# smu-ivpl/FastInterCU-VVC

Hardware: AMD Instinct MI355X
Metric: CU-inferences/sec (batch 4096, 128x128) (higher is better)
Workload: dtype f16 (fp32 accumulate)

## Files before the change

fastintercu-vvc_amd/csrc/mlt_chain_kernel.inc:

```
template <class T> __device__ __forceinline__ T karg_reload(size_t off) {
  const __attribute__((address_space(4))) char *ka = (const __attribute__((address_space(4))) char *)__builtin_amdgcn_kernarg_segment_ptr();
  asm volatile("" : "+s"(ka));
  return *(const __attribute__((address_space(4))) T *)(ka + off);
}
#define KARG(type, member) karg_reload<type>(offsetof(ChainArgs, member))

template <int C, int HL, int SPW_L, int WCB, int WPB, int WAVES_C, int WAVES_P, int GT, int RB, int FD, int MINW, int NCONV, bool SPLIT_ROLES, bool S2 = false, bool KEEP = true, bool OOBZ = false, bool W2 = false, bool LO8 = false>
__global__ __launch_bounds__(64 * WAVES_C * WAVES_P, MINW) void chain_kernel(const ChainArgs a) {
  constexpr int KC = 64, NCHUNK = C / KC, KS = KC / 16, SLOTS = KC / 8, TAPS = 9, NG = (TAPS + GT - 1) / GT, GT_LAST = TAPS - (NG - 1) * GT;
  constexpr int CBT = WCB * WAVES_C, CT = 32 * CBT, NPASS = C / CT, NW = WAVES_C * WAVES_P;
  constexpr int H = 1 << HL, HW = H * H, M = HW << SPW_L;
  static_assert(C % CT == 0 && NPASS <= 2 && M == 32 * WAVES_P * WPB && HW >= 32 && C % KC == 0, "tiling");
  static_assert(GT_LAST == GT || RB == 2, "a shorter last tap group issues fewer ring pieces: only with the uncounted vmcnt(0) wait of a 2-deep ring");
  constexpr int WP = (W2 && !LO8) ? 2 : 1, WPLANE = GT * KS * CBT * 1024;
  constexpr int WLO8 = LO8 ? GT * CBT * 2048 : 0;
  constexpr int WCHUNK = WP * WPLANE + WLO8, NPIECE = WCHUNK / 1024, NBUF = RB, PFD = RB - 1;
  static_assert(!W2 || (!S2 && GT_LAST == GT), "hi+lo weights: no stride-2 front conv, whole tap groups");
  static_assert(!LO8 || (W2 && KS == 4 && FD == 1 && KEEP && NCHUNK > 1), "FP8 lo plane: 64-channel chunks, fragment reads one item ahead, stage forms");
  constexpr int REGION8 = LO8 ? M * KC : 0, ACT8 = NCHUNK * REGION8;
  constexpr int NWR = SPLIT_ROLES ? NW / 2 : NW, NWP = SPLIT_ROLES ? NW - NWR : NW, WP0 = SPLIT_ROLES ? NWR : 0;
  constexpr int PPWR = (NPIECE + NWR - 1) / NWR;
  constexpr int REGION = M * KC * 2, ACT = NCHUNK * REGION, RPIECE = REGION / 1024, PPR = (RPIECE + NWP - 1) / NWP;
  constexpr int A8BASE = ACT + NBUF * WCHUNK;
  static_assert(A8BASE + ACT8 <= 160 * 1024, "LDS");
  static_assert(RB >= 2 && RB <= 4, "ring depth");
  static_assert(SPLIT_ROLES || RB == 2, "unified issue waits with vmcnt(0)");
  static_assert(!S2 || KEEP, "the whole-stage variant keeps sc / b0 in registers");
  static_assert(FD >= 1 && FD <= 3 && FD * (WP * WCB + WPB) + (LO8 ? 2 * (WCB > WPB ? WCB : WPB) : 0) <= 15, "fragment prefetch distance");
  static_assert((WP - 1) * WPLANE + ((GT * KS - 1) * CBT + WCB - 1) * 1024 < 65536 && WPLANE + WLO8 < 65536, "fragment offsets are ds_read immediates");
  constexpr int CIN = C / 2, HIN = 2 * H, KCS = 16, NCS = CIN / KCS, TAPS_S = 10, NS = S2 ? NPASS * NCS : 0;
  constexpr int NCH = NCONV * NPASS * NCHUNK * NG;
  constexpr int WSTEP_S = TAPS_S * CBT * 1024, NPIECE_S = WSTEP_S / 1024;
  constexpr int PRS = 2 * H + 1, PCW = 2 * H + 1, PPS = PRS * PCW, PPIX = PPS << SPW_L;
  constexpr int PBYTES = (PPIX * KCS * 2 + 1023) / 1024 * 1024, PPIECE = PBYTES / 1024;
  constexpr int SOFF0 = ACT + 8 * 1024, SOFF1 = ACT + WCHUNK + 8 * 1024;
  constexpr int NPB = 3 * PBYTES <= SOFF0 ? 3 : 2, PLA = NPB - 1;
  auto pbuf = [](int i) { return NPB == 3 ? i % 3 : (i + 1) & 1; };
  static_assert(!S2 || (NPB == 3 ? (NS - 1) % 3 == 0 : (NS - 1) % 2 == 1), "S2: the last stride-2 step must read patch buffer 0");
  static_assert(!S2 || (SPLIT_ROLES && RB == 2 && NS % 2 == 0 && NCH % 2 == 0 && (NCS - 1) % 2 == 1), "S2: step parities");
  static_assert(!S2 || (2 * PBYTES <= SOFF0 && SOFF0 + WSTEP_S <= ACT + WCHUNK && SOFF1 + WSTEP_S <= 160 * 1024), "S2: LDS layout");

  extern __shared__ __attribute__((aligned(16))) char smem[];
  char *ring = smem + ACT;
  const uint32_t lds0 = (uint32_t)(uintptr_t)LDS_PTR(smem);
  const int tid = threadIdx.x, lane = tid & 63;
  const int wave = __builtin_amdgcn_readfirstlane(tid >> 6);
  const int wc = wave % WAVES_C, wp = wave / WAVES_C;
  const int p = lane & 31, h = lane >> 5;
  const bool ring_wave = wave < NWR, patch_wave = wave >= WP0;
  const int lane16 = lane * 16;

  const int pr = p < 4 ? p : p < 12 ? p + 12 : p < 16 ? p - 8 : p < 20 ? p + 8 : p < 28 ? p - 12 : p;
  int mj[WPB], pj[WPB];
// ... 23 lines not shown
  };

  const int ntiles = (a.n + (1 << SPW_L) - 1) >> SPW_L;
  int t = blockIdx.x;
  const int tstep = gridDim.x;
  if (t >= ntiles) return;

  int steps_to_issue = ((ntiles - 1 - t) / tstep + 1) * (NS + NCH);
  int r_pos = 0, r_cv = 0, r_ps = 0, r_ci = 0, r_gi = 0, ahead = 0;
  int slot_wr = 0;
  auto issue_ring = [&]() {
    if (steps_to_issue <= 0) return;
    const bool s_step = S2 && r_pos < NS;
    if (ring_wave) {
      if (s_step) {
      } else {
        const char *wsrc = (const char *)(r_cv == 0 ? a.cv[0].w : r_cv == 1 ? a.cv[1].w : a.cv[NCONV > 2 ? 2 : 1].w);
        const char *src = wsrc + (size_t)((r_ps * NCHUNK + r_ci) * TAPS + r_gi * GT) * (KS * CBT * 1024);
        char *dst = ring + slot_wr * WCHUNK;
        const int npiece = (GT_LAST != GT && r_gi == NG - 1) ? GT_LAST * KS * CBT : NPIECE;
        const size_t wlo = W2 ? (r_cv == 0 ? a.cv[0].w_lo_off : r_cv == 1 ? a.cv[1].w_lo_off : a.cv[NCONV > 2 ? 2 : 1].w_lo_off) : 0;
#pragma unroll
        for (int k = 0; k < PPWR; ++k) {
          int pi = wave + k * NWR;
          pi = pi < npiece ? pi : npiece - 1;
          const int pl = W2 ? pi / (WPLANE / 1024) : 0, pw = W2 ? pi - pl * (WPLANE / 1024) : pi;
          if (LO8 && pl) glds16(wsrc + wlo + (size_t)((r_ps * NCHUNK + r_ci) * TAPS + r_gi * GT) * (CBT * 2048) + pw * 1024 + lane16, dst + pi * 1024);
          else glds16(src + (pl ? wlo : 0) + pw * 1024 + lane16, dst + pi * 1024);
        }
      }
    }
    if (s_step) {
      const char *src = (const char *)a.s2_w + (size_t)r_pos * WSTEP_S;
      char *dst = smem + ((r_pos & 1) ? SOFF1 : SOFF0);
#pragma unroll
      for (int k = 0; k < (NPIECE_S + NW - 1) / NW; ++k) {
        const int pi = wave + k * NW;
        if (pi < NPIECE_S) glds16(src + pi * 1024 + lane16, dst + pi * 1024);
      }
    }
    --steps_to_issue;
    ++ahead;
    if (!s_step) {
      if (++slot_wr == NBUF) slot_wr = 0;
      if (++r_gi == NG) { r_gi = 0; if (++r_ci == NCHUNK) { r_ci = 0; if (++r_ps == NPASS) { r_ps = 0; if (++r_cv == NCONV) r_cv = 0; } } }
    }
    if (++r_pos == NS + NCH) r_pos = 0;
  };
  constexpr int PPW = (PPIECE + NW - 1) / NW;
  uint32_t pvo[S2 ? PPW : 1];
  if constexpr (S2) {
#pragma unroll
    for (int k = 0; k < PPW; ++k) {
      const int piece = wave + k * NW;
      const int it = piece * 64 + lane, qS = it >> 1, pos = it & 1;
      const int sl = pos ^ ((qS >> 3) & 1);
      const int sm = qS / PPS, rem = qS - sm * PPS, r = rem / PCW, kk = rem - r * PCW;
      const int ri = r - 1, ci = kk <= H ? 2 * kk - 1 : 2 * (kk - H - 1);
      const bool live = qS < PPIX && ri >= 0 && ri < HIN && ci >= 0 && ci < HIN;
      const uint32_t off = a.x_c16 ? ((ri * HIN + ci) * KCS + sl * 8) * 2
// ... 126 lines not shown
      if (patch_wave) asm volatile("s_waitcnt vmcnt(0)" ::: "memory");
      PHC_MARK(1);
      asm volatile("s_barrier" ::: "memory");
      PHC_MARK(0);
    }
    if constexpr (S2) {
      asm volatile("s_waitcnt vmcnt(0)\n\ts_barrier" ::: "memory");
      PHC_MARK(0);
      int bS[WPB];
#pragma unroll
      for (int j = 0; j < WPB; ++j) bS[j] = ((pj[j] >> (2 * HL)) * PRS + 2 * ((pj[j] >> HL) & (H - 1))) * PCW + (pj[j] & (H - 1));
      auto put_t = [&](int pass, int i, int j, int qq, uint4v w) {
        const int cb = pass * CT + (wc * WCB + i) * 32 + 16 * qq + 8 * h;
        *(uint4v *)(smem + (cb / KC) * REGION + pj[j] * (KC * 2) + ((((cb % KC) / 8) ^ swz(pj[j])) << 4)) = w;
      };
      static_for<NPASS>([&](auto kp) {
        constexpr int ps = decltype(kp)::value;
        float16v acc[WCB][WPB], accs[WCB][WPB];
#pragma unroll
        for (int i = 0; i < WCB; ++i)
#pragma unroll
          for (int j = 0; j < WPB; ++j)
#pragma unroll
            for (int r = 0; r < 16; ++r) { acc[i][j][r] = 0.f; accs[i][j][r] = 0.f; }
#pragma unroll 1
        for (int chunk = 0; chunk < NCS; ++chunk) {
          const int si = ps * NCS + chunk;
          if (si >= 1 && si + PLA < NS) patch_dma(t, si + PLA);
          issue_ring();
          {
// ... 75 lines not shown
              for (int qq = 0; qq < 2; ++qq) put_t(0, i, j, qq, hold0[i][j][qq]);
        }
      });
      asm volatile("s_waitcnt lgkmcnt(0)\n\ts_barrier" ::: "memory");
      PHC_MARK(3);
    }

    static_for<NCONV>([&](auto kc) {
      constexpr int cvi = decltype(kc)::value;
      constexpr bool lastc = cvi == NCONV - 1;
      const ChainConv &cv = a.cv[cvi];
      constexpr int RES = NCONV == 3 ? (cvi == 0 ? (S2 ? 2 : 1) : cvi == 2 ? (KEEP ? 2 : 1) : 0) : (cvi == 1 ? 1 : 0);
      constexpr bool SAVE = KEEP && NCONV == 3 && cvi == 0;
      constexpr bool RES_LATE = !KEEP;
      uint4v hold[WCB][WPB][2];
      static_for<NPASS>([&](auto kp) {
        constexpr int ps = decltype(kp)::value;
        constexpr bool last = lastc && ps == NPASS - 1;
        float16v acc[WCB][WPB];
#pragma unroll
        for (int i = 0; i < WCB; ++i)
#pragma unroll
          for (int j = 0; j < WPB; ++j)
#pragma unroll
            for (int r = 0; r < 16; ++r) acc[i][j][r] = 0.f;
        uint4v resv[WCB][WPB][2];

#pragma unroll 1
        for (int chunk = 0; chunk < NCHUNK; ++chunk) {
          const uint32_t pl = lds0 + chunk * REGION;
// ... 157 lines not shown
          };
#pragma unroll 1
          for (int g = 0; g < (GT_LAST != GT ? NG - 1 : NG); ++g) do_step(g, std::integral_constant<int, GT * KS>{});
          if constexpr (GT_LAST != GT) do_step(NG - 1, std::integral_constant<int, GT_LAST * KS>{});
        }
        if constexpr (lastc) {
          if constexpr (last) {
            if constexpr (S2) {
              if (has_next) {
#pragma unroll
                for (int i = 0; i < NPB; ++i) patch_dma(t + tstep, i);
              }
            } else if (has_next) dma_region(t + tstep, NCHUNK - 1);
          }
          if constexpr (S2 || !KEEP) out_index_late();
          auto std_epi = [&]() {
          float4v bq[WCB][4], bsq[1][4];
#pragma unroll
          for (int i = 0; i < WCB; ++i) {
            if constexpr (PBIAS) bias_rows(pb_cv[cvi][ps], i, bq[i]);
            else {
#pragma unroll
              for (int q = 0; q < 4; ++q) bq[i][q] = *(const float4v *)(cv.bias + ps * CT + (wc * WCB + i) * 32 + 4 * h + 8 * q);
            }
          }
          ConvArgs ea{};
          ea.y = a.y; ea.gap = a.gap; ea.gap_slots = a.gap_slots; ea.gap_l = a.gap_l; ea.acc_scale = cv.acc_scale; ea.relu = 1;
          ea.y_c16 = a.y_c16; ea.hout_l = HL;
          ea.res = RES ? (const void *)a.x : nullptr;
          float16v acc_sc[1][1];
          uint4v resl[1][1][2];
          if constexpr (RES == 2) {
#pragma unroll
            for (int i = 0; i < WCB; ++i)
#pragma unroll
              for (int j = 0; j < WPB; ++j)
#pragma unroll
                for (int qq = 0; qq < 2; ++qq) resv[i][j][qq] = keep[ps][i][j][qq];
          }
          int he = h, pe = p;
          asm volatile("" : "+v"(he), "+v"(pe));
          conv_epilogue<C, CT, WCB, WPB, false, 1>(ea, ps, wc, he, pe, opix, gidx, acc, acc_sc, bq, bsq, resv, resl);
          };
          auto blk_epi = [&]() {
            ConvArgs ea{};
            ea.y = KARG(void *, y); ea.gap = KARG(float *, gap); ea.gap_slots = KARG(int, gap_slots); ea.gap_l = KARG(int, gap_l);
            ea.acc_scale = KARG(float, cv[cvi].acc_scale); ea.relu = 1;
            ea.y_c16 = KARG(int, y_c16); ea.hout_l = HL;
            ea.res = RES ? (const void *)ea.y : nullptr;
            float16v acc_sc[1][1];
            uint4v resl[1][1][2];
            float4v bsq[1][4];
#pragma unroll
            for (int i = 0; i < WCB; ++i) {
              float4v bq1[1][4];
              bias_rows(pb_cv[cvi][ps], i, bq1[0]);
              if (i) out_index_late();
              int he = h, pe = p;
              asm volatile("" : "+v"(he), "+v"(pe));
              conv_epilogue<C, CT, 1, WPB, false, 1>(ea, ps, wc * WCB + i, he, pe, opix, gidx, reinterpret_cast<float16v(&)[1][WPB]>(acc[i]), acc_sc, bq1, bsq,
                                                     reinterpret_cast<const uint4v(&)[1][WPB][2]>(resv[i]), resl);
            }
          };
          if constexpr (!KEEP && PBIAS) blk_epi();
          else std_epi();
          PHC_MARK(6 + 3 * cvi);
        } else {
          _Float16 *yb0 = nullptr;
          if constexpr (!KEEP) yb0 = (_Float16 *)KARG(void *, cv[cvi].y);
          const int hm = KEEP ? h : (int)__builtin_amdgcn_mbcnt_hi(~0u, __builtin_amdgcn_mbcnt_lo(~0u, 0u)) >> 5;
          auto put = [&](int pass, int i, int j, int qq, uint4v w) {
            const int cb = pass * CT + (wc * WCB + i) * 32 + 16 * qq + 8 * hm;
            *(uint4v *)(smem + (cb / KC) * REGION + pj[j] * (KC * 2) + ((((cb % KC) / 8) ^ swz(pj[j])) << 4)) = w;
            if constexpr (LO8) {
              uint32_t d0, d1;
              cvt_frag_fp8(*(const half8 *)&w, d0, d1);
              typedef uint32_t uint2v __attribute__((ext_vector_type(2)));
              *(uint2v *)(smem + A8BASE + (cb / KC) * REGION8 + pj[j] * KC + (((((cb % KC) >> 4) ^ ((pj[j] >> 2) & 3)) << 4) | (cb & 8))) = uint2v{d0, d1};
            }
          };
// ... 28 lines not shown
              for (int i = 0; i < WCB; ++i)
#pragma unroll
                for (int j = 0; j < WPB; ++j)
#pragma unroll
                  for (int qq = 0; qq < 2; ++qq) put(0, i, j, qq, hold[i][j][qq]);
            }
            asm volatile("s_waitcnt lgkmcnt(0)\n\ts_barrier" ::: "memory");
          }
          PHC_MARK(6 + 3 * cvi);
        }
      });
    });
  }
  PHC_FLUSH((C == 256 ? 2 : 0) + (S2 ? 1 : 0));
}
```

fastintercu-vvc_amd/csrc/mlt_dispatch.cpp:

```cpp
#include "mlt_runtime.h"

const char *tuning_env(const char *name) {
  const char *e = std::getenv("MLT_TUNING");
  return (e && e[0] == '1') ? std::getenv(name) : nullptr;
}

const Tuning &tuning() {
  static const Tuning t = [] {
    auto num = [](const char *name, long dflt) { const char *e = tuning_env(name); return e ? std::atol(e) : dflt; };
    auto on = [](const char *name) { return tuning_env(name) != nullptr; };
    auto cap = [&](const char *name) { const long v = num(name, 0); return (int)(v > 0 ? v : 256); };
    Tuning u{};
    u.debug_dump_dir = tuning_env("MLT_DEBUG_DUMP_DIR");
    u.xl_kill = (int)num("MLT_XL_KILL", 0); u.xl_kill_layer = (int)num("MLT_XL_KILL_LAYER", -1);
    u.lat_pixels = num("MLT_LAT_PIXELS", 16384L);
    u.no_exact_lat = on("MLT_NO_EXACT_LAT"); u.exact_patch_big = !on("MLT_EXACT_PATCH_64K");
    u.wg_cap = cap("MLT_WG_CAP"); u.wg_cap0 = cap("MLT_WG_CAP0"); u.wg_cap1 = cap("MLT_WG_CAP1"); u.wg_cap2 = cap("MLT_WG_CAP2");
    u.l0_mfma32 = on("MLT_L0_MFMA32"); u.l1_mfma32 = !on("MLT_L1_MFMA16");
    u.no_block_fusion = on("MLT_NO_BLOCK_FUSION");
    u.no_chain = on("MLT_NO_CHAIN") || u.no_block_fusion; u.no_chain_s2 = on("MLT_NO_CHAIN_S2"); u.no_c16 = on("MLT_NO_C16"); u.chain64 = !on("MLT_NO_CHAIN64");
    u.no_l0_s5 = on("MLT_NO_L0_S5");
    u.no_xs_handoff = on("MLT_NO_XS_HANDOFF") || u.debug_dump_dir != nullptr;
    u.l0_stream_min = on("MLT_NO_L0_STREAM") ? 0 : (int)num("MLT_L0_STREAM_MIN", 128);
    u.l1_stream_min = on("MLT_NO_L1_STREAM") ? 0 : (int)num("MLT_L1_STREAM_MIN", 128);
    u.guard_wait_mode = on("MLT_GUARD_SPIN_WAIT") ? 1 : on("MLT_GUARD_BLOCKING_WAIT") ? 2 : 0;
    u.no_small_mix = on("MLT_NO_SMALL_MIX"); u.no_mag_guard = on("MLT_NO_MAG_GUARD");
    u.no_graph = on("MLT_NO_GRAPH") || u.debug_dump_dir != nullptr;
    return u;
  }();
  return t;
}

namespace {

int gap_slots(int hw) { return hw >= 32 ? hw / 32 : 1; }

size_t ws_per_cu(const mlt::Model &m, int S, bool some_exact = false) {
// ... 264 lines not shown
  const int grid_x = a.ntiles > wg_cap ? wg_cap : a.ntiles;
  char name[48];
  std::snprintf(name, sizeof name, "block_s1_32_h%d(conv1+conv2)", h);
  const double px = (double)n * h * h;
  Launch L{ctx};
  hipEvent_t e0 = nullptr, e1 = nullptr;
  int rc = L.prof_begin(name, 2.0 * px * 32 * 32 * 9 * 2, px * 32 * 2 * 2 + 2.0 * 18 * 1024, e0, e1, w2 ? "hi+lo weights" : "single pass");
  if (rc) return rc;
  plan_note(ctx, {{"x", x}, {"y", y}}, {{"grid", grid_x}});
  LAUNCH_TRY(ctx, mlt_launch_block32(a, w2, grid_x, ctx->stream));
  if ((rc = L.prof_end(e1))) return rc;
  return debug_dump(ctx, name, y, (size_t)px * 32 * 2);
}

int run_chain3(mlt_ctx *ctx, const mlt::Block &B0, const mlt::Block &B1, int n, int h, const void *t, const void *sc, void *y, float *gap,
               const void *s2_in, bool x_c16, bool y_c16, void *b0_hbm, bool sc_c16) {
  const int c = B0.conv2.cout;
  ChainArgs a{};
  a.x = s2_in ? s2_in : t; a.nconv = 3; a.y = y; a.gap = gap; a.n = n; a.zero = ctx->zero_page;
  a.x_c16 = x_c16 ? 1 : 0; a.y_c16 = y_c16 ? 1 : 0; a.res0_c16 = sc_c16 ? 1 : 0;
  const mlt::PackedConv *pcs[3] = {&B0.conv2, &B1.conv1, &B1.conv2};
  const bool w2 = B0.conv2.w2;
  for (int k = 0; k < 3; ++k) {
    a.cv[k].w = pcs[k]->d_w; a.cv[k].bias = pcs[k]->d_bias; a.cv[k].acc_scale = pcs[k]->acc_scale; a.cv[k].relu = 1;
    a.cv[k].w_lo_off = pcs[k]->plane_halves * 2;
    a.cv[k].lo8_scale = 0x01010101 * ((127 - pcs[k]->lo8_exp) & 0xFF);
  }
  a.cv[0].res_mode = s2_in ? 2 : 1; a.cv[0].res = sc; a.cv[0].save = 1; a.cv[2].res_mode = 2;
  if (c == 64) {
    a.cv[0].save = 0; a.cv[0].y = b0_hbm; a.cv[2].res_mode = 1; a.cv[2].res = b0_hbm;
  }
// ... 4 lines not shown
  const int hw = h * h;
  a.gap_slots = gap_slots(hw); a.gap_l = hw >= 32 ? 5 : ilog2(hw);
  const int wg_cap = tuning().wg_cap;
  const int spw = c == 256 ? 2 : 1;
  const int ntiles = (n + spw - 1) / spw;
  const int grid_x = ntiles > wg_cap ? wg_cap : ntiles;
  char name[48];
  std::snprintf(name, sizeof name, s2_in ? "stage_%d_h%d(s2+sc,conv2,conv1,conv2)" : "chain3_s1_%d_h%d(conv2+conv1+conv2)", c, h);
  const double px = (double)n * hw;
  const double flops = 3.0 * 2.0 * px * c * c * 9 + (s2_in ? 2.0 * px * c * (c / 2) * 10 : 0.0);
  const double bytes = (s2_in ? px * 4 * (c / 2) * 2 : px * c * 2 * 2) + (y ? px * c * 2 : 0.0) + 3.0 * (double)B0.conv2.w.size() * 2 +
                       (s2_in ? (double)B0.conv1_s2c.w.size() * 2 : 0.0);
  Launch L{ctx};
  hipEvent_t e0 = nullptr, e1 = nullptr;
  char variant[96];
  std::snprintf(variant, sizeof variant, "%s%s%s%s%s", w2 ? "hi+lo weights" : "single pass", x_c16 ? ", x chunk-major" : "", sc_c16 ? ", sc chunk-major" : "", y_c16 ? ", y chunk-major" : "",
                gap ? ", GAP" : "");
  int rc = L.prof_begin(name, flops, bytes, e0, e1, variant);
  if (rc) return rc;
  plan_note(ctx, {{"x", a.x}, {"sc", s2_in ? nullptr : sc}, {"y", y}, {"gap", gap}, {"b0", c == 64 ? b0_hbm : nullptr}}, {{"grid", grid_x}});
  LAUNCH_TRY(ctx, mlt_launch_chain(c, h, s2_in != nullptr, ctx->lds_oob_zero, w2, a, grid_x, ctx->stream));
  if ((rc = L.prof_end(e1))) return rc;
  if (y && (rc = debug_dump(ctx, name, y, (size_t)px * c * 2))) return rc;
  return MLT_OK;
}

int run_layer1_stream(mlt_ctx *ctx, const mlt::Block &B0, const mlt::Block &B1, int n, const void *t, const void *sc, void *y, float *gap, bool y_c16, const mlt::PackedConv *c5xs) {
  Layer1Args a{};
  const bool xs = c5xs != nullptr;
  if (xs) { a.w_sc = c5xs->d_w; a.bias_sc = c5xs->d_bias_sc; a.scale_sc = c5xs->acc_scale; }
  a.t = t; a.sc = sc; a.y = y; a.y_c16 = y_c16 ? 1 : 0; a.gap = gap; a.gap_slots = gap_slots(32 * 32); a.n = n;
  const mlt::PackedConv *pcs[3] = {&B0.conv2, &B1.conv1, &B1.conv2};
  for (int k = 0; k < 3; ++k) { a.w[k] = pcs[k]->d_w; a.bias[k] = pcs[k]->d_bias; a.scale[k] = pcs[k]->acc_scale; }
  const int wg_cap = tuning().wg_cap1;
  const int grid_x = n > wg_cap ? wg_cap : n;
  const double px = (double)n * 32 * 32;
// ... 69 lines not shown
      bool sc_c16 = false;
      if (s == 0) add(PlanStep::STEM5, 0);
      else if (chain_s2) {}
      else if (s == 1 && l0_front) sc_c16 = true;
      else {
        sc_c16 = chain && m.planes[s] == 64 && !tn.no_c16 && !ms.exact;
        add(PlanStep::CONV_S2, s).sc_c16 = sc_c16;
      }
      if (chain) {
        const bool out_c16 = !last && !tn.no_c16 && wants_s2(s + 1);
        const mlt::PackedConv &q2 = mt.blocks[s][0].conv2;
        const bool stream = s == 1 && !chain_s2 && m.planes[s] == 64 && ho == 32 && sc_c16 && !mt.w2 && !mt.exact && (cls & CLS_L1_STREAM) &&
                            q2.taps == 9 && q2.kc == 64 && q2.ct == 64 && !last;
        PlanStep &st = add(stream ? PlanStep::LAYER1_STREAM : PlanStep::CHAIN, s);
        st.inside_s2 = chain_s2; st.x_c16 = cur_c16; st.sc_c16 = sc_c16; st.y_c16 = out_c16;
        if (stream && l0_front && l0_front_step >= 0 && !tn.no_xs_handoff && !tn.l0_mfma32 && tn.l1_mfma32) st.xs = P[(size_t)l0_front_step].xs = true;
        cur_c16 = out_c16;
        continue;
      }
      add(PlanStep::CONV_B0C2, s);
    }
    if (s == 0 && !mt.exact && ho >= 32 && !tn.no_block_fusion) { add(PlanStep::BLOCK32, 0); continue; }
    add(PlanStep::CONV_B1C1, s);
    PlanStep &st = add(PlanStep::CONV_B1C2, s);
    st.y_c16 = !last && !tn.no_c16 && wants_s2(s + 1);
    cur_c16 = st.y_c16;
  }
  add(PlanStep::HEADS, m.n_stages - 1);
  return P;
}
// ... 66 lines not shown
      break;
    case PlanStep::STEM_BLOCK:
      rc = run_stem_block(ctx, ms, n, S, io.pl, pool[2], go.d_flat, go.flat_is_clear);
      break;
    case PlanStep::STEM5:
      rc = run_stem5(ctx, ms.stem, n, S, io.pl, pool[0], pool[1], lo_st);
      break;
    case PlanStep::CONV_S2:
      cv.x = cur; cv.y = pool[0]; cv.y_sc = pool[1]; cv.relu = true;
      cv.x_lo = in_has_lo ? lo_in : 0; cv.y_lo = lo_st; cv.ysc_lo = lo_st;
      cv.ysc_c16 = ps.sc_c16;
      rc = run_conv(ctx, ms.blocks[s][0].conv1, n, h, cv, &hh);
      break;
    case PlanStep::CHAIN:
      rc = run_chain3(ctx, mt.blocks[s][0], mt.blocks[s][1], n, ho, pool[0], pool[1], last ? nullptr : outs[s], gaps[s], ps.inside_s2 ? cur : nullptr,
                      ps.x_c16, ps.y_c16, pool[2], ps.sc_c16);
      break;
    case PlanStep::LAYER1_STREAM:
      rc = run_layer1_stream(ctx, mt.blocks[s][0], mt.blocks[s][1], n, pool[0], pool[1], outs[s], gaps[s], ps.y_c16, ps.xs ? &c.model_of(1, 0).blocks[1][0].conv1 : nullptr);
      break;
    case PlanStep::CONV_B0C2:
      cv.x = pool[0]; cv.y = pool[2]; cv.res = pool[1]; cv.relu = true;
      cv.x_lo = cv.y_lo = cv.res_lo = lo_st;
      if (s > 0 && ex1 && !ex0) cv.x_lo = cv.res_lo = 0;
      rc = run_conv(ctx, (s == 0 ? ms : mt).blocks[s][0].conv2, n, ho, cv, &hh);
      break;
    case PlanStep::BLOCK32:
      rc = run_block32(ctx, mt.blocks[0][1], n, ho, pool[2], outs[0]);
      break;
    case PlanStep::CONV_B1C1:
      cv.x = pool[2]; cv.y = pool[3]; cv.relu = true;
// ... 97 lines not shown
```

fastintercu-vvc_amd/csrc/mlt_kernels.h:

```cpp
#pragma once
#include <hip/hip_runtime.h>
#include <stdint.h>

#define MLT_MAX_HEADS_K 4
#define MLT_MAX_LOGITS_K 16
#define MLT_FLAT_RANGE 6
#define MLT_FLAT_EXACT_SHIFT 16

struct ConvArgs {
  const void *x;
  void *y;
  const void *w;
  const float *bias;
  const void *res;
  const void *zero;
  int n;
  int ntiles;
  int hin_l, hout_l;
  int tw_l, th_l, spw_l;
  int ph, pw, rp, half;
  uint32_t pw_magic, ph_magic, rp_magic;
  int patch_bytes;
  int relu;
  int y_c16;
// ... 99 lines not shown
  const void *s2_w;
  const float *s2_bias, *s2_bias_sc;
  float s2_scale;
  const void *zero;
  ChainConv cv[3];
  int nconv;
  void *y;
  int y_c16;
  int x_c16;
  int res0_c16;
  float *gap;
  int gap_slots, gap_l;
  int n;
};
hipError_t mlt_launch_chain(int c, int h, bool with_s2, bool oob_zero, bool w2, const ChainArgs &a, int grid_x, hipStream_t st);
bool mlt_chain_supported(int c, int h);
hipError_t mlt_probe_lds_oob(int *d_ok, hipStream_t st);
bool mlt_stage_supported(int c, int h);

struct DecisionRec {
  int32_t split_mode, raw_mode;
  float confidence, margin;
  int32_t level_mode[MLT_MAX_HEADS_K];
  float level_conf[MLT_MAX_HEADS_K];
};
#define MLT_CONF_BAND_FRAC 0.75f

#define MLT_MAX_CAND_K 6
struct CandRec {
  uint32_t mask;
// ... 220 lines not shown
```

fastintercu-vvc_amd/csrc/mlt_kernels.hip:

```cpp
#include <hip/hip_runtime.h>
#include <hip/hip_fp16.h>
#include <stdint.h>

#include <atomic>
#include <utility>

#include "mlt_kernels.h"

#ifndef CFG_ASM_PIPE
#define CFG_ASM_PIPE 1
#endif
#ifndef CFG_S2_BIAS_EARLY
#define CFG_S2_BIAS_EARLY 1
#endif
#ifndef CFG_DMA_SPREAD
#define CFG_DMA_SPREAD 5
#endif
#ifndef CFG_RING_FD16
#define CFG_RING_FD16 1
#endif
#ifndef CFG_RING_RES_EARLY
#define CFG_RING_RES_EARLY 1
#endif
#ifndef CFG_BIAS_EARLY
// ... 613 lines not shown
      return launch_chain_t(chain_kernel<128, 4, 0, 2, 2, 2, 4, 3, 2, CFG_CHAIN_FD, 2, 3, true, true, true, false>, once[8], a, grid_x, 512, lds, st);
    }
    if (a.nconv == 3) return launch_chain_t(chain_kernel<128, 4, 0, 2, 2, 2, 4, 3, 2, CFG_CHAIN_FD, 2, 3, CFG_CHAIN_SPLIT != 0>, once[0], a, grid_x, 512, lds, st);
    if (a.nconv == 2) return launch_chain_t(chain_kernel<128, 4, 0, 2, 2, 2, 4, 3, 2, CFG_CHAIN_FD, 2, 2, CFG_CHAIN_SPLIT != 0>, once[1], a, grid_x, 512, lds, st);
  }
  if (c == 256 && h == 8) {
    if (with_s2 && a.nconv == 3) {
      if (oob_zero) return launch_chain_t(chain_kernel<256, 3, 1, 2, 1, 2, 4, 3, 2, CFG_CHAIN_FD, 2, 3, true, true, true, true>, once[5], a, grid_x, 512, lds, st);
      return launch_chain_t(chain_kernel<256, 3, 1, 2, 1, 2, 4, 3, 2, CFG_CHAIN_FD, 2, 3, true, true, true, false>, once[9], a, grid_x, 512, lds, st);
    }
    if (a.nconv == 3) return launch_chain_t(chain_kernel<256, 3, 1, 2, 1, 2, 4, 3, 2, CFG_CHAIN_FD, 2, 3, CFG_CHAIN_SPLIT != 0>, once[2], a, grid_x, 512, lds, st);
    if (a.nconv == 2) return launch_chain_t(chain_kernel<256, 3, 1, 2, 1, 2, 4, 3, 2, CFG_CHAIN_FD, 2, 2, CFG_CHAIN_SPLIT != 0>, once[3], a, grid_x, 512, lds, st);
  }
  return hipErrorInvalidValue;
}

hipError_t mlt_launch_stem5(const Stem5Args &a, int nsplit, int grid_x, int lds, hipStream_t st) {
  if (nsplit == 3) hipLaunchKernelGGL(stem5_kernel<3>, dim3(grid_x), dim3(256), lds, st, a);
  else if (nsplit == 2) hipLaunchKernelGGL(stem5_kernel<2>, dim3(grid_x), dim3(256), lds, st, a);
  else hipLaunchKernelGGL(stem5_kernel<1>, dim3(grid_x), dim3(256), lds, st, a);
  return hipGetLastError();
}

hipError_t mlt_launch_block32(const Block32Args &a, bool w2, int grid_x, hipStream_t st) {
  static DeviceOnce once[2];
  if (w2) {
    constexpr int lds = (12 * 36 + 10 * 34) * 80 + 4 * 18 * 1024;
    if (hipError_t e = ensure_big_lds(block32_kernel<3, true>, once[1]); e != hipSuccess) return e;
    hipLaunchKernelGGL((block32_kernel<3, true>), dim3(grid_x), dim3(512), lds, st, a);
    return hipGetLastError();
// ... 156 lines not shown
```

fastintercu-vvc_amd/csrc/mlt_runtime.h:

```cpp
#pragma once
#include <hip/hip_runtime.h>

#include <algorithm>
#include <chrono>
#include <cmath>
#include <cstddef>
#include <cstdio>
#include <cstdlib>
#include <cstring>
#include <map>
#include <tuple>
#include <mutex>
#include <string>
#include <thread>
#include <vector>

#include "../../include/mltcnn.h"
#include "mlt_kernels.h"
#include "mlt_layout.h"
#include "mlt_model.h"
#include "mlt_tier_search.h"

const char *tuning_env(const char *name);

struct Tuning {
  const char *debug_dump_dir;
  int xl_kill, xl_kill_layer;
  long lat_pixels;
  bool no_exact_lat;
  bool exact_patch_big;
  int wg_cap, wg_cap0, wg_cap1, wg_cap2;
  bool l0_mfma32, l1_mfma32;
  bool no_chain, no_chain_s2, no_c16, chain64, no_block_fusion, no_l0_s5;
  bool no_xs_handoff;
  int l0_stream_min, l1_stream_min;
  int guard_wait_mode;
  bool no_small_mix, no_mag_guard, no_graph;
};
const Tuning &tuning();

inline int size_index(int size) {
  switch (size) {
    case 128: return 0;
    case 64: return 1;
    case 32: return 2;
    case 16: return 3;
    default: return -1;
  }
}
// ... 14 lines not shown
    STEM_BLOCK,
    STEM5,
    CONV_S2,
    CHAIN,
    LAYER1_STREAM,
    CONV_B0C2,
    BLOCK32,
    CONV_B1C1,
    CONV_B1C2,
    HEADS
  } kind;
  int8_t s = 0;
  bool front = false;
  bool xs = false;
  bool inside_s2 = false;
  bool x_c16 = false;
  bool sc_c16 = false;
  bool y_c16 = false;
};
using NetPlan = std::vector<PlanStep>;
using PlanKey = std::tuple<const void *, const void *, const void *, unsigned, unsigned, unsigned>;

struct SizeState {
  bool enabled = false, loaded = false;
  std::map<PlanKey, NetPlan> plans;
  bool exact = false;
  bool w2 = false;
  unsigned w2_mask = 0;
  unsigned w2_units = 0;
  unsigned x_mask = 0;
// ... 258 lines not shown
```

Baseline: 1.034 million.

## Add wide 256-channel stage kernel computing both cout passes per wave

Adds a WIDE variant of the chain kernel for the 256-channel 8x8 stage with the stride-2 front conv. Each wave accumulates both output-channel passes at once, so every activation/patch fragment read from LDS feeds twice as many MFMAs, and the number of ring steps and barriers per stage is halved. Weight staging is reorganized into half-chunks covering both passes with 6-item groups. The cost is doubled accumulator register pressure, which can lower occupancy or cause spills, plus new dispatch plumbing with an env opt-out.

After: 1.052 million (median of 6 runs). +1.7%, better.

```diff
diff --git a/fastintercu-vvc_amd/csrc/mlt_chain_kernel.inc b/fastintercu-vvc_amd/csrc/mlt_chain_kernel.inc
--- a/fastintercu-vvc_amd/csrc/mlt_chain_kernel.inc
+++ b/fastintercu-vvc_amd/csrc/mlt_chain_kernel.inc
@@ -5,8 +5,8 @@
 }
 #define KARG(type, member) karg_reload<type>(offsetof(ChainArgs, member))
 
-template <int C, int HL, int SPW_L, int WCB, int WPB, int WAVES_C, int WAVES_P, int GT, int RB, int FD, int MINW, int NCONV, bool SPLIT_ROLES, bool S2 = false, bool KEEP = true, bool OOBZ = false, bool W2 = false, bool LO8 = false>
-__global__ __launch_bounds__(64 * WAVES_C * WAVES_P, MINW) void chain_kernel(const ChainArgs a) {
+template <int C, int HL, int SPW_L, int WCB, int WPB, int WAVES_C, int WAVES_P, int GT, int RB, int FD, int MINW, int NCONV, bool SPLIT_ROLES, bool S2 = false, bool KEEP = true, bool OOBZ = false, bool W2 = false, bool LO8 = false, bool WIDE = false>
+__device__ __forceinline__ void chain_body(const ChainArgs &a) {
   constexpr int KC = 64, NCHUNK = C / KC, KS = KC / 16, SLOTS = KC / 8, TAPS = 9, NG = (TAPS + GT - 1) / GT, GT_LAST = TAPS - (NG - 1) * GT;
   constexpr int CBT = WCB * WAVES_C, CT = 32 * CBT, NPASS = C / CT, NW = WAVES_C * WAVES_P;
   constexpr int H = 1 << HL, HW = H * H, M = HW << SPW_L;
@@ -36,7 +36,12 @@
   constexpr int SOFF0 = ACT + 8 * 1024, SOFF1 = ACT + WCHUNK + 8 * 1024;
   constexpr int NPB = 3 * PBYTES <= SOFF0 ? 3 : 2, PLA = NPB - 1;
   auto pbuf = [](int i) { return NPB == 3 ? i % 3 : (i + 1) & 1; };
-  static_assert(!S2 || (NPB == 3 ? (NS - 1) % 3 == 0 : (NS - 1) % 2 == 1), "S2: the last stride-2 step must read patch buffer 0");
+  static_assert(!S2 || WIDE || (NPB == 3 ? (NS - 1) % 3 == 0 : (NS - 1) % 2 == 1), "S2: the last stride-2 step must read patch buffer 0");
+  constexpr int WI = 6, NG6 = TAPS * KS / WI, WHALF = WCHUNK / 2, TH = TAPS_S / 2, WHALF_S = WSTEP_S / 2;
+  static_assert(!WIDE || (NPASS == 2 && S2 && KEEP && OOBZ && !W2 && NCONV == 3 && GT == 3 && KS == 4 && FD == 1 && 2 * WI == GT * KS && NG6 * WI == TAPS * KS),
+                "WIDE: the whole 256-channel stage, conv padding from beyond the LDS, fragment reads one item ahead");
+  static_assert(!WIDE || (NPB == 3 && NCS >= 3 && 3 * PBYTES <= ACT), "WIDE: three patch buffers, all below the chain's ring slot 0");
+  static_assert(!WIDE || (WHALF + ((WI - 1) * CBT + WCB - 1) * 1024 < 65536 && WHALF_S + ((TH - 1) * CBT + WCB - 1) * 1024 < 65536), "WIDE: fragment offsets are ds_read immediates");
   static_assert(!S2 || (SPLIT_ROLES && RB == 2 && NS % 2 == 0 && NCH % 2 == 0 && (NCS - 1) % 2 == 1), "S2: step parities");
   static_assert(!S2 || (2 * PBYTES <= SOFF0 && SOFF0 + WSTEP_S <= ACT + WCHUNK && SOFF1 + WSTEP_S <= 160 * 1024), "S2: LDS layout");
 
@@ -90,6 +95,15 @@
     const bool s_step = S2 && r_pos < NS;
     if (ring_wave) {
       if (s_step) {
+      } else if constexpr (WIDE) {
+        const char *wsrc = (const char *)(r_cv == 0 ? a.cv[0].w : r_cv == 1 ? a.cv[1].w : a.cv[2].w);
+        char *dst = ring + slot_wr * WCHUNK;
+#pragma unroll
+        for (int k = 0; k < PPWR; ++k) {
+          const int pi = wave + k * NWR, ps = pi / (NPIECE / 2), pw = pi - ps * (NPIECE / 2);
+          static_assert(!WIDE || NPIECE % NWR == 0, "every ring wave issues PPWR pieces");
+          glds16(wsrc + (size_t)((ps * NCHUNK + r_ci) * (TAPS * KS) + r_gi * WI) * (CBT * 1024) + pw * 1024 + lane16, dst + pi * 1024);
+        }
       } else {
         const char *wsrc = (const char *)(r_cv == 0 ? a.cv[0].w : r_cv == 1 ? a.cv[1].w : a.cv[NCONV > 2 ? 2 : 1].w);
         const char *src = wsrc + (size_t)((r_ps * NCHUNK + r_ci) * TAPS + r_gi * GT) * (KS * CBT * 1024);
@@ -112,14 +126,20 @@
 #pragma unroll
       for (int k = 0; k < (NPIECE_S + NW - 1) / NW; ++k) {
         const int pi = wave + k * NW;
-        if (pi < NPIECE_S) glds16(src + pi * 1024 + lane16, dst + pi * 1024);
+        if constexpr (WIDE) {
+          const int ps = pi / (NPIECE_S / 2), pw = pi - ps * (NPIECE_S / 2);
+          const char *srcw = (const char *)a.s2_w + (size_t)((ps * NCS + (r_pos >> 1)) * TAPS_S + (r_pos & 1) * TH) * (CBT * 1024);
+          if (pi < NPIECE_S) glds16(srcw + pw * 1024 + lane16, dst + pi * 1024);
+        } else if (pi < NPIECE_S) glds16(src + pi * 1024 + lane16, dst + pi * 1024);
       }
     }
     --steps_to_issue;
     ++ahead;
     if (!s_step) {
       if (++slot_wr == NBUF) slot_wr = 0;
-      if (++r_gi == NG) { r_gi = 0; if (++r_ci == NCHUNK) { r_ci = 0; if (++r_ps == NPASS) { r_ps = 0; if (++r_cv == NCONV) r_cv = 0; } } }
+      if constexpr (WIDE) {
+        if (++r_gi == NG6) { r_gi = 0; if (++r_ci == NCHUNK) { r_ci = 0; if (++r_cv == NCONV) r_cv = 0; } }
+      } else if (++r_gi == NG) { r_gi = 0; if (++r_ci == NCHUNK) { r_ci = 0; if (++r_ps == NPASS) { r_ps = 0; if (++r_cv == NCONV) r_cv = 0; } } }
     }
     if (++r_pos == NS + NCH) r_pos = 0;
   };
@@ -276,6 +296,93 @@
         const int cb = pass * CT + (wc * WCB + i) * 32 + 16 * qq + 8 * h;
         *(uint4v *)(smem + (cb / KC) * REGION + pj[j] * (KC * 2) + ((((cb % KC) / 8) ^ swz(pj[j])) << 4)) = w;
       };
+      if constexpr (WIDE) {
+        float16v acc[NPASS][WCB][WPB], accs[NPASS][WCB][WPB];
+#pragma unroll
+        for (int ps = 0; ps < NPASS; ++ps)
+#pragma unroll
+          for (int i = 0; i < WCB; ++i)
+#pragma unroll
+            for (int j = 0; j < WPB; ++j)
+#pragma unroll
+              for (int r = 0; r < 16; ++r) { acc[ps][i][j][r] = 0.f; accs[ps][i][j][r] = 0.f; }
+#pragma unroll 1
+        for (int chunk = 0; chunk < NCS; ++chunk) {
+          const uint32_t pb = lds0 + pbuf(chunk) * PBYTES;
+          static_for<2>([&](auto hc) {
+            constexpr int hf = decltype(hc)::value;
+            if constexpr (hf == 0) {
+              if (chunk >= 1 && chunk + PLA < NCS) patch_dma(t, chunk + PLA);
+            }
+            issue_ring();
+            {
+              const uint32_t wb = lds0 + (hf ? SOFF1 : SOFF0) + (wc * WCB) * 1024 + lane16;
+              half8 fa[2][NPASS][WCB], fb[2][WPB];
+              auto issue = [&](auto ic) {
+                constexpr int tl = decltype(ic)::value, sl = tl & 1, tt = TH * hf + tl;
+                constexpr int te = tt == 9 ? 4 : tt, dy = te / 3, dx = te % 3;
+                constexpr int off = dy * PCW + (dx == 1 ? H + 1 : dx / 2);
+                static_for<NPASS * WCB>([&](auto ii) {
+                  constexpr int ps = decltype(ii)::value / WCB, i = decltype(ii)::value % WCB;
+                  lds_read128<ps * WHALF_S + (tl * CBT + i) * 1024>(fa[sl][ps][i], wb);
+                });
+                static_for<WPB>([&](auto jj) {
+                  constexpr int j = decltype(jj)::value;
+                  const int qS = bS[j] + off;
+                  lds_read128<0>(fb[sl][j], pb + qS * (KCS * 2) + ((h ^ ((qS >> 3) & 1)) << 4));
+                });
+              };
+              issue(std::integral_constant<int, 0>{});
+              static_for<TH>([&](auto ic) {
+                constexpr int tl = decltype(ic)::value, sl = tl & 1, tt = TH * hf + tl;
+                if constexpr (tl + 1 < TH) issue(std::integral_constant<int, tl + 1>{});
+                lds_wait<(tl + 1 < TH ? NPASS * WCB + WPB : 0)>();
+#pragma unroll
+                for (int ps = 0; ps < NPASS; ++ps)
+#pragma unroll
+                  for (int i = 0; i < WCB; ++i) lds_touch(fa[sl][ps][i]);
+#pragma unroll
+                for (int j = 0; j < WPB; ++j) lds_touch(fb[sl][j]);
+#pragma unroll
+                for (int ps = 0; ps < NPASS; ++ps)
+#pragma unroll
+                  for (int i = 0; i < WCB; ++i)
+#pragma unroll
+                    for (int j = 0; j < WPB; ++j) {
+                      if constexpr (tt == 9) accs[ps][i][j] = __builtin_amdgcn_mfma_f32_32x32x16_f16(fa[sl][ps][i], fb[sl][j], accs[ps][i][j], 0, 0, 0);
+                      else acc[ps][i][j] = __builtin_amdgcn_mfma_f32_32x32x16_f16(fa[sl][ps][i], fb[sl][j], acc[ps][i][j], 0, 0, 0);
+                    }
+              });
+            }
+            PHC_MARK(1);
+            asm volatile("s_waitcnt vmcnt(0)\n\ts_barrier" ::: "memory");
+            PHC_MARK(2);
+            --ahead;
+          });
+        }
+        static_for<NPASS>([&](auto kp) {
+          constexpr int ps = decltype(kp)::value;
+#pragma unroll
+          for (int i = 0; i < WCB; ++i) {
+            float4v b1[4], bs[4];
+            bias_rows(pb_t[ps], i, b1);
+            bias_rows(pb_sc[ps], i, bs);
+#pragma unroll
+            for (int j = 0; j < WPB; ++j)
+              static_for<2>([&](auto qc) {
+                constexpr int qq = decltype(qc)::value;
+                half4 ht[2], hc[2];
+                const half4 none{};
+                ht[0] = act_quad<2 * qq>(acc[ps][i][j], a.s2_scale, b1[2 * qq], false, none, true);
+                ht[1] = act_quad<2 * qq + 1>(acc[ps][i][j], a.s2_scale, b1[2 * qq + 1], false, none, true);
+                hc[0] = act_quad<2 * qq>(accs[ps][i][j], a.s2_scale, bs[2 * qq], false, none, false);
+                hc[1] = act_quad<2 * qq + 1>(accs[ps][i][j], a.s2_scale, bs[2 * qq + 1], false, none, false);
+                keep[ps][i][j][qq] = pair16(hc[0], hc[1]);
+                put_t(ps, i, j, qq, pair16(ht[0], ht[1]));
+              });
+          }
+        });
+      } else
       static_for<NPASS>([&](auto kp) {
         constexpr int ps = decltype(kp)::value;
         float16v acc[WCB][WPB], accs[WCB][WPB];
@@ -381,6 +488,141 @@
       constexpr bool SAVE = KEEP && NCONV == 3 && cvi == 0;
       constexpr bool RES_LATE = !KEEP;
       uint4v hold[WCB][WPB][2];
+      auto std_epi = [&](auto kp, float16v(&acc)[WCB][WPB], uint4v(&resv)[WCB][WPB][2]) {
+        constexpr int ps = decltype(kp)::value;
+        float4v bq[WCB][4], bsq[1][4];
+#pragma unroll
+        for (int i = 0; i < WCB; ++i) {
+          if constexpr (PBIAS) bias_rows(pb_cv[cvi][ps], i, bq[i]);
+          else {
+#pragma unroll
+            for (int q = 0; q < 4; ++q) bq[i][q] = *(const float4v *)(cv.bias + ps * CT + (wc * WCB + i) * 32 + 4 * h + 8 * q);
+          }
+        }
+        ConvArgs ea{};
+        ea.y = a.y; ea.gap = a.gap; ea.gap_slots = a.gap_slots; ea.gap_l = a.gap_l; ea.acc_scale = cv.acc_scale; ea.relu = 1;
+        ea.y_c16 = a.y_c16; ea.hout_l = HL;
+        ea.res = RES ? (const void *)a.x : nullptr;
+        float16v acc_sc[1][1];
+        uint4v resl[1][1][2];
+        if constexpr (RES == 2) {
+#pragma unroll
+          for (int i = 0; i < WCB; ++i)
+#pragma unroll
+            for (int j = 0; j < WPB; ++j)
+#pragma unroll
+              for (int qq = 0; qq < 2; ++qq) resv[i][j][qq] = keep[ps][i][j][qq];
+        }
+        int he = h, pe = p;
+        asm volatile("" : "+v"(he), "+v"(pe));
+        conv_epilogue<C, CT, WCB, WPB, false, 1>(ea, ps, wc, he, pe, opix, gidx, acc, acc_sc, bq, bsq, resv, resl);
+      };
+      if constexpr (WIDE) {
+        float16v acc[NPASS][WCB][WPB];
+#pragma unroll
+        for (int ps = 0; ps < NPASS; ++ps)
+#pragma unroll
+          for (int i = 0; i < WCB; ++i)
+#pragma unroll
+            for (int j = 0; j < WPB; ++j)
+#pragma unroll
+              for (int r = 0; r < 16; ++r) acc[ps][i][j][r] = 0.f;
+#pragma unroll 1
+        for (int chunk = 0; chunk < NCHUNK; ++chunk) {
+          const uint32_t pl = lds0 + chunk * REGION;
+#pragma unroll 1
+          for (int g = 0; g < NG; ++g) {
+            static_for<2>([&](auto hc) {
+              constexpr int hf = decltype(hc)::value;
+              issue_ring();
+              {
+                const uint32_t wb = lds0 + ACT + slot_rd * WCHUNK + (wc * WCB) * 1024 + lane16;
+                half8 fa[2][NPASS][WCB], fb[2][WPB];
+                uint32_t rowa[WPB], hs[WPB];
+                auto issue = [&](auto ic) {
+                  constexpr int item = decltype(ic)::value, il = item - WI * hf, sl = item & 1, tt = item / KS, ks = item % KS;
+                  if constexpr (ks == 0 || il == 0) {
+                    const int tp = g * GT + tt, dy = tp / 3, dx = tp - dy * 3;
+#pragma unroll
+                    for (int j = 0; j < WPB; ++j) {
+                      const int yy = ((pj[j] >> HL) & (H - 1)) + dy - 1, xx = (pj[j] & (H - 1)) + dx - 1;
+                      const bool ok = (unsigned)yy < (unsigned)H && (unsigned)xx < (unsigned)H;
+                      const int q = ok ? pj[j] + (dy - 1) * H + (dx - 1) : pj[j];
+                      rowa[j] = ok ? pl + q * (KC * 2) : 0x100000u;
+                      hs[j] = (h * 16) ^ (swz(q) << 4);
+                    }
+                  }
+                  static_for<NPASS * WCB>([&](auto ii) {
+                    constexpr int ps = decltype(ii)::value / WCB, i = decltype(ii)::value % WCB;
+                    lds_read128<ps * WHALF + (il * CBT + i) * 1024>(fa[sl][ps][i], wb);
+                  });
+                  static_for<WPB>([&](auto jj) { lds_read128<0>(fb[sl][decltype(jj)::value], rowa[decltype(jj)::value] + (hs[decltype(jj)::value] ^ (ks * 32))); });
+                };
+                issue(std::integral_constant<int, WI * hf>{});
+                static_for<WI>([&](auto ic) {
+                  constexpr int il = decltype(ic)::value, item = WI * hf + il, sl = item & 1;
+                  if constexpr (il + 1 < WI) issue(std::integral_constant<int, item + 1>{});
+                  lds_wait<(il + 1 < WI ? NPASS * WCB + WPB : 0)>();
+#pragma unroll
+                  for (int ps = 0; ps < NPASS; ++ps)
+#pragma unroll
+                    for (int i = 0; i < WCB; ++i) lds_touch(fa[sl][ps][i]);
+#pragma unroll
+                  for (int j = 0; j < WPB; ++j) lds_touch(fb[sl][j]);
+#pragma unroll
+                  for (int ps = 0; ps < NPASS; ++ps)
+#pragma unroll
+                    for (int i = 0; i < WCB; ++i)
+#pragma unroll
+                      for (int j = 0; j < WPB; ++j) acc[ps][i][j] = __builtin_amdgcn_mfma_f32_32x32x16_f16(fa[sl][ps][i], fb[sl][j], acc[ps][i][j], 0, 0, 0);
+                });
+              }
+              PHC_MARK(4 + 3 * cvi);
+              if (ring_wave) asm volatile("s_waitcnt vmcnt(0)" ::: "memory");
+              asm volatile("s_barrier" ::: "memory");
+              PHC_MARK(5 + 3 * cvi);
+              --ahead;
+              slot_rd ^= 1;
+            });
+          }
+        }
+        if constexpr (lastc) {
+          if (has_next) {
+#pragma unroll
+            for (int i = 0; i < NPB; ++i) patch_dma(t + tstep, i);
+          }
+          out_index_late();
+          static_for<NPASS>([&](auto kp) {
+            uint4v resv[WCB][WPB][2];
+            std_epi(kp, acc[decltype(kp)::value], resv);
+          });
+          PHC_MARK(6 + 3 * cvi);
+        } else {
+          static_for<NPASS>([&](auto kp) {
+            constexpr int ps = decltype(kp)::value;
+#pragma unroll
+            for (int i = 0; i < WCB; ++i) {
+              float4v bi[4];
+              bias_rows(pb_cv[cvi][ps], i, bi);
+#pragma unroll
+              for (int j = 0; j < WPB; ++j)
+                static_for<2>([&](auto qc) {
+                  constexpr int qq = decltype(qc)::value;
+                  half4 ra{}, rb{}, hq[2];
+                  if constexpr (RES != 0) unpair16(keep[ps][i][j][qq], ra, rb);
+                  hq[0] = act_quad<2 * qq>(acc[ps][i][j], cv.acc_scale, bi[2 * qq], RES != 0, ra, true);
+                  hq[1] = act_quad<2 * qq + 1>(acc[ps][i][j], cv.acc_scale, bi[2 * qq + 1], RES != 0, rb, true);
+                  const uint4v w = pair16(hq[0], hq[1]);
+                  if constexpr (SAVE) keep[ps][i][j][qq] = w;
+                  const int cb = ps * CT + (wc * WCB + i) * 32 + 16 * qq + 8 * h;
+                  *(uint4v *)(smem + (cb / KC) * REGION + pj[j] * (KC * 2) + ((((cb % KC) / 8) ^ swz(pj[j])) << 4)) = w;
+                });
+            }
+          });
+          asm volatile("s_waitcnt lgkmcnt(0)\n\ts_barrier" ::: "memory");
+          PHC_MARK(6 + 3 * cvi);
+        }
+      } else
       static_for<NPASS>([&](auto kp) {
         constexpr int ps = decltype(kp)::value;
         constexpr bool last = lastc && ps == NPASS - 1;
@@ -568,34 +810,6 @@
             } else if (has_next) dma_region(t + tstep, NCHUNK - 1);
           }
           if constexpr (S2 || !KEEP) out_index_late();
-          auto std_epi = [&]() {
-          float4v bq[WCB][4], bsq[1][4];
-#pragma unroll
-          for (int i = 0; i < WCB; ++i) {
-            if constexpr (PBIAS) bias_rows(pb_cv[cvi][ps], i, bq[i]);
-            else {
-#pragma unroll
-              for (int q = 0; q < 4; ++q) bq[i][q] = *(const float4v *)(cv.bias + ps * CT + (wc * WCB + i) * 32 + 4 * h + 8 * q);
-            }
-          }
-          ConvArgs ea{};
-          ea.y = a.y; ea.gap = a.gap; ea.gap_slots = a.gap_slots; ea.gap_l = a.gap_l; ea.acc_scale = cv.acc_scale; ea.relu = 1;
-          ea.y_c16 = a.y_c16; ea.hout_l = HL;
-          ea.res = RES ? (const void *)a.x : nullptr;
-          float16v acc_sc[1][1];
-          uint4v resl[1][1][2];
-          if constexpr (RES == 2) {
-#pragma unroll
-            for (int i = 0; i < WCB; ++i)
-#pragma unroll
-              for (int j = 0; j < WPB; ++j)
-#pragma unroll
-                for (int qq = 0; qq < 2; ++qq) resv[i][j][qq] = keep[ps][i][j][qq];
-          }
-          int he = h, pe = p;
-          asm volatile("" : "+v"(he), "+v"(pe));
-          conv_epilogue<C, CT, WCB, WPB, false, 1>(ea, ps, wc, he, pe, opix, gidx, acc, acc_sc, bq, bsq, resv, resl);
-          };
           auto blk_epi = [&]() {
             ConvArgs ea{};
             ea.y = KARG(void *, y); ea.gap = KARG(float *, gap); ea.gap_slots = KARG(int, gap_slots); ea.gap_l = KARG(int, gap_l);
@@ -617,7 +831,7 @@
             }
           };
           if constexpr (!KEEP && PBIAS) blk_epi();
-          else std_epi();
+          else std_epi(kp, acc, resv);
           PHC_MARK(6 + 3 * cvi);
         } else {
           _Float16 *yb0 = nullptr;
@@ -676,3 +890,11 @@
   }
   PHC_FLUSH((C == 256 ? 2 : 0) + (S2 ? 1 : 0));
 }
+
+template <int C, int HL, int SPW_L, int WCB, int WPB, int WAVES_C, int WAVES_P, int GT, int RB, int FD, int MINW, int NCONV, bool SPLIT_ROLES, bool S2 = false, bool KEEP = true, bool OOBZ = false, bool W2 = false, bool LO8 = false>
+__global__ __launch_bounds__(64 * WAVES_C * WAVES_P, MINW) void chain_kernel(const ChainArgs a) {
+  chain_body<C, HL, SPW_L, WCB, WPB, WAVES_C, WAVES_P, GT, RB, FD, MINW, NCONV, SPLIT_ROLES, S2, KEEP, OOBZ, W2, LO8>(a);
+}
+__global__ __launch_bounds__(512, 2) void stage256_wide_kernel(const ChainArgs a) {
+  chain_body<256, 3, 1, 2, 1, 2, 4, 3, 2, 1, 2, 3, true, true, true, true, false, false, true>(a);
+}
diff --git a/fastintercu-vvc_amd/csrc/mlt_dispatch.cpp b/fastintercu-vvc_amd/csrc/mlt_dispatch.cpp
--- a/fastintercu-vvc_amd/csrc/mlt_dispatch.cpp
+++ b/fastintercu-vvc_amd/csrc/mlt_dispatch.cpp
@@ -21,6 +21,7 @@
     u.no_chain = on("MLT_NO_CHAIN") || u.no_block_fusion; u.no_chain_s2 = on("MLT_NO_CHAIN_S2"); u.no_c16 = on("MLT_NO_C16"); u.chain64 = !on("MLT_NO_CHAIN64");
     u.no_l0_s5 = on("MLT_NO_L0_S5");
     u.no_xs_handoff = on("MLT_NO_XS_HANDOFF") || u.debug_dump_dir != nullptr;
+    u.no_stage256_wide = on("MLT_NO_STAGE256_WIDE");
     u.l0_stream_min = on("MLT_NO_L0_STREAM") ? 0 : (int)num("MLT_L0_STREAM_MIN", 128);
     u.l1_stream_min = on("MLT_NO_L1_STREAM") ? 0 : (int)num("MLT_L1_STREAM_MIN", 128);
     u.guard_wait_mode = on("MLT_GUARD_SPIN_WAIT") ? 1 : on("MLT_GUARD_BLOCKING_WAIT") ? 2 : 0;
@@ -315,7 +316,7 @@
 }
 
 int run_chain3(mlt_ctx *ctx, const mlt::Block &B0, const mlt::Block &B1, int n, int h, const void *t, const void *sc, void *y, float *gap,
-               const void *s2_in, bool x_c16, bool y_c16, void *b0_hbm, bool sc_c16) {
+               const void *s2_in, bool x_c16, bool y_c16, void *b0_hbm, bool sc_c16, bool wide) {
   const int c = B0.conv2.cout;
   ChainArgs a{};
   a.x = s2_in ? s2_in : t; a.nconv = 3; a.y = y; a.gap = gap; a.n = n; a.zero = ctx->zero_page;
@@ -350,12 +351,16 @@
   Launch L{ctx};
   hipEvent_t e0 = nullptr, e1 = nullptr;
   char variant[96];
-  std::snprintf(variant, sizeof variant, "%s%s%s%s%s", w2 ? "hi+lo weights" : "single pass", x_c16 ? ", x chunk-major" : "", sc_c16 ? ", sc chunk-major" : "", y_c16 ? ", y chunk-major" : "",
+  std::snprintf(variant, sizeof variant, "%s%s%s%s%s%s", wide ? "both cout passes per wave, " : "", w2 ? "hi+lo weights" : "single pass", x_c16 ? ", x chunk-major" : "", sc_c16 ? ", sc chunk-major" : "", y_c16 ? ", y chunk-major" : "",
                 gap ? ", GAP" : "");
   int rc = L.prof_begin(name, flops, bytes, e0, e1, variant);
   if (rc) return rc;
   plan_note(ctx, {{"x", a.x}, {"sc", s2_in ? nullptr : sc}, {"y", y}, {"gap", gap}, {"b0", c == 64 ? b0_hbm : nullptr}}, {{"grid", grid_x}});
-  LAUNCH_TRY(ctx, mlt_launch_chain(c, h, s2_in != nullptr, ctx->lds_oob_zero, w2, a, grid_x, ctx->stream));
+  if (wide) {
+    LAUNCH_TRY(ctx, c == 256 && h == 8 && s2_in && !w2 && ctx->lds_oob_zero ? mlt_launch_stage256_wide(a, grid_x, ctx->stream) : hipErrorInvalidValue);
+  } else {
+    LAUNCH_TRY(ctx, mlt_launch_chain(c, h, s2_in != nullptr, ctx->lds_oob_zero, w2, a, grid_x, ctx->stream));
+  }
   if ((rc = L.prof_end(e1))) return rc;
   if (y && (rc = debug_dump(ctx, name, y, (size_t)px * c * 2))) return rc;
   return MLT_OK;
@@ -455,6 +460,7 @@
                             q2.taps == 9 && q2.kc == 64 && q2.ct == 64 && !last;
         PlanStep &st = add(stream ? PlanStep::LAYER1_STREAM : PlanStep::CHAIN, s);
         st.inside_s2 = chain_s2; st.x_c16 = cur_c16; st.sc_c16 = sc_c16; st.y_c16 = out_c16;
+        st.wide = chain_s2 && m.planes[s] == 256 && ho == 8 && ctx->lds_oob_zero && !tn.no_stage256_wide;
         if (stream && l0_front && l0_front_step >= 0 && !tn.no_xs_handoff && !tn.l0_mfma32 && tn.l1_mfma32) st.xs = P[(size_t)l0_front_step].xs = true;
         cur_c16 = out_c16;
         continue;
@@ -551,7 +557,7 @@
       break;
     case PlanStep::CHAIN:
       rc = run_chain3(ctx, mt.blocks[s][0], mt.blocks[s][1], n, ho, pool[0], pool[1], last ? nullptr : outs[s], gaps[s], ps.inside_s2 ? cur : nullptr,
-                      ps.x_c16, ps.y_c16, pool[2], ps.sc_c16);
+                      ps.x_c16, ps.y_c16, pool[2], ps.sc_c16, ps.wide);
       break;
     case PlanStep::LAYER1_STREAM:
       rc = run_layer1_stream(ctx, mt.blocks[s][0], mt.blocks[s][1], n, pool[0], pool[1], outs[s], gaps[s], ps.y_c16, ps.xs ? &c.model_of(1, 0).blocks[1][0].conv1 : nullptr);
diff --git a/fastintercu-vvc_amd/csrc/mlt_kernels.h b/fastintercu-vvc_amd/csrc/mlt_kernels.h
--- a/fastintercu-vvc_amd/csrc/mlt_kernels.h
+++ b/fastintercu-vvc_amd/csrc/mlt_kernels.h
@@ -137,6 +137,7 @@
   int n;
 };
 hipError_t mlt_launch_chain(int c, int h, bool with_s2, bool oob_zero, bool w2, const ChainArgs &a, int grid_x, hipStream_t st);
+hipError_t mlt_launch_stage256_wide(const ChainArgs &a, int grid_x, hipStream_t st);
 bool mlt_chain_supported(int c, int h);
 hipError_t mlt_probe_lds_oob(int *d_ok, hipStream_t st);
 bool mlt_stage_supported(int c, int h);
diff --git a/fastintercu-vvc_amd/csrc/mlt_kernels.hip b/fastintercu-vvc_amd/csrc/mlt_kernels.hip
--- a/fastintercu-vvc_amd/csrc/mlt_kernels.hip
+++ b/fastintercu-vvc_amd/csrc/mlt_kernels.hip
@@ -651,6 +651,11 @@
   }
   return hipErrorInvalidValue;
 }
+hipError_t mlt_launch_stage256_wide(const ChainArgs &a, int grid_x, hipStream_t st) {
+  static DeviceOnce once;
+  if (a.nconv != 3 || !a.s2_w) return hipErrorInvalidValue;
+  return launch_chain_t(stage256_wide_kernel, once, a, grid_x, 512, 160 * 1024, st);
+}
 
 hipError_t mlt_launch_stem5(const Stem5Args &a, int nsplit, int grid_x, int lds, hipStream_t st) {
   if (nsplit == 3) hipLaunchKernelGGL(stem5_kernel<3>, dim3(grid_x), dim3(256), lds, st, a);
diff --git a/fastintercu-vvc_amd/csrc/mlt_runtime.h b/fastintercu-vvc_amd/csrc/mlt_runtime.h
--- a/fastintercu-vvc_amd/csrc/mlt_runtime.h
+++ b/fastintercu-vvc_amd/csrc/mlt_runtime.h
@@ -33,6 +33,7 @@
   bool l0_mfma32, l1_mfma32;
   bool no_chain, no_chain_s2, no_c16, chain64, no_block_fusion, no_l0_s5;
   bool no_xs_handoff;
+  bool no_stage256_wide;
   int l0_stream_min, l1_stream_min;
   int guard_wait_mode;
   bool no_small_mix, no_mag_guard, no_graph;
@@ -77,6 +78,7 @@
   bool front = false;
   bool xs = false;
   bool inside_s2 = false;
+  bool wide = false;
   bool x_c16 = false;
   bool sc_c16 = false;
   bool y_c16 = false;
```
